# imulki/serenade

Measured on AMD Instinct MI355X. Metric: mel frames/sec converted (UNet ODE + vocoder), 80x1024, higher is better.
Workload: dtype f32

## Files before the change

serenade_amd/csrc/resunit_f32.hip:

```cpp
#include <hip/hip_runtime.h>

#include "common.h"
#include "conv_common.h"
#include "serenade_hip.h"

namespace {

constexpr int HALO_MAX = 50;
constexpr int NTH = 512;

typedef unsigned u32x4r __attribute__((ext_vector_type(4)));

struct FDivR {
  uint32_t mul, shift;
};
__device__ __forceinline__ int fdivr(const int n, const FDivR d) {
  return (int)(((uint64_t)(uint32_t)n * d.mul) >> d.shift);
}

template <int C_>
struct UCfg {
  static constexpr int C = C_, CH = C / 32;
  static constexpr int BMI = C == 32 ? 256 : 128;
  static constexpr int A_ROWS = BMI + HALO_MAX + 2;
  static constexpr int A_PLANE = A_ROWS * 144;
  static constexpr int A_BYTES = CH * A_PLANE;
  static constexpr int UNIT = C * 144;
  static constexpr int G = 9216 / UNIT >= 2 ? 2 : 1;
  static constexpr int STAGE = G * UNIT;
  static constexpr int SMEM = A_BYTES + 2 * STAGE;
  static constexpr int F4R = C / 4, RSTEP = NTH / F4R;
  static constexpr int A_LD = (A_ROWS * F4R + NTH - 1) / NTH;
  static_assert(G * C * 8 == NTH, "one 16-B weight piece per thread per stage");
};

template <class R>
__global__ __launch_bounds__(NTH, 4) void resunit_f32_kernel(const SrnResUnitParams p, const int tiles_per_z,
                                                             const int n_tiles, const FDivR d_tpz) {
  constexpr int C = R::C, CH = R::CH, BMI = R::BMI, G = R::G;
  extern __shared__ __attribute__((aligned(16))) unsigned char smem_u[];
  unsigned char* const sA = smem_u;
  unsigned char* const sW = smem_u + R::A_BYTES;

  const int tid = threadIdx.x;
  const int lane = tid & 63;
  const int wave = __builtin_amdgcn_readfirstlane(tid >> 6);
  const int li = lane & 31;
  const int lh = lane >> 5;
  const int k = p.k, dil = p.dilation, T = p.T;
  const int p2 = (k - 1) / 2, p1 = p2 * dil;
  const int BMo = BMI - (k - 1);
  const int hr = BMI + (k - 1) * dil;
  const int U = k * CH;
  const int S = (U + G - 1) / G;
  const float slope = p.slope;

  const int w_n = (tid % (C * 8)) >> 3;
  const int w_g = tid / (C * 8);
  const int w_voff = w_n * (k * C * 4) + w_g * 128 + (tid & 7) * 16;
  const int w_dst = (w_g * C + w_n) * 144 + (tid & 7) * 16;
  const int w_bytes = C * k * C * 4;
  const __amdgpu_buffer_rsrc_t rs_w1 = __builtin_amdgcn_make_buffer_rsrc(const_cast<float*>(p.w1), 0, w_bytes, 0x00020000);
  const __amdgpu_buffer_rsrc_t rs_w2 = __builtin_amdgcn_make_buffer_rsrc(const_cast<float*>(p.w2), 0, w_bytes, 0x00020000);
  u32x4r wr;
  auto w_load = [&](const int j) {
    if (j >= S) wr = __builtin_amdgcn_raw_buffer_load_b128(rs_w2, w_voff, (j - S) * G * 128, 0);
    else wr = __builtin_amdgcn_raw_buffer_load_b128(rs_w1, w_voff, j * G * 128, 0);
  };
  auto w_store = [&](const int buf) {
    *reinterpret_cast<u32x4r*>(sW + buf * R::STAGE + w_dst) = wr;
  };

  constexpr int A_LD = R::A_LD, F4R = R::F4R, RSTEP = R::RSTEP;
  const int a_f4 = tid % F4R;
  const int a_r0 = tid / F4R;
  const int a_voff = (a_r0 * C + a_f4 * 4) * 4;
  const int a_dst0 = (a_f4 >> 3) * R::A_PLANE + a_r0 * 144 + (a_f4 & 7) * 16;
  u32x4r pa[A_LD];
  auto load_a = [&](const int tile) {
    const int z = fdivr(tile, d_tpz);
    const int t0 = (tile - z * tiles_per_z) * BMo;
    const __amdgpu_buffer_rsrc_t rs_x =
        __builtin_amdgcn_make_buffer_rsrc(const_cast<float*>(p.x + (int64_t)z * p.x_bs), 0, T * C * 4, 0x00020000);
    const int v0 = a_voff + (t0 - p2 - p1) * (C * 4);
#pragma unroll
    for (int j = 0; j < A_LD; ++j) pa[j] = __builtin_amdgcn_raw_buffer_load_b128(rs_x, v0 + j * (RSTEP * C * 4), 0, 0);
  };
  auto stage_a = [&]() {
#pragma unroll
    for (int j = 0; j < A_LD; ++j) {
      if (a_r0 + RSTEP * j < hr) {
        float4 v = __builtin_bit_cast(float4, pa[j]);
        v.x = fmaxf(v.x, v.x * slope);
        v.y = fmaxf(v.y, v.y * slope);
        v.z = fmaxf(v.z, v.z * slope);
        v.w = fmaxf(v.w, v.w * slope);
        *reinterpret_cast<float4*>(sA + a_dst0 + j * RSTEP * 144) = v;
      }
    }
  };

  const int wm0 = (C == 64 ? (wave & 3) : wave) * 32;
  const int ng0 = C == 64 ? (wave >> 2) : 0;
  const int fa_lane = (wm0 + li) * 144 + 16 * lh;
  const int fb_lane = R::A_BYTES + (ng0 * 32 + li) * 144 + 16 * lh;
  f32x16 acc;
  auto zero_acc = [&]() {
#pragma unroll
    for (int r = 0; r < 16; ++r) acc[r] = 0.f;
  };

  auto compute = [&](const int buf, const int u0, const int step) {
#pragma unroll
    for (int g = 0; g < G; ++g) {
      const int u = u0 + g;
      if (u >= U) break;
      const int tap = u / CH;
      const int c = u - tap * CH;
      const float* a = reinterpret_cast<const float*>(smem_u + (fa_lane + (c * R::A_PLANE + tap * step * 144)));
      const float* b = reinterpret_cast<const float*>(smem_u + (fb_lane + (buf * R::STAGE + g * C * 144)));
#pragma unroll
      for (int kk = 0; kk < 4; ++kk) {
        const float4 af = *reinterpret_cast<const float4*>(a + kk * 8);
        const float4 bf = *reinterpret_cast<const float4*>(b + kk * 8);
        acc = __builtin_amdgcn_mfma_f32_32x32x2f32(af.x, bf.x, acc, 0, 0, 0);
        acc = __builtin_amdgcn_mfma_f32_32x32x2f32(af.y, bf.y, acc, 0, 0, 0);
        acc = __builtin_amdgcn_mfma_f32_32x32x2f32(af.z, bf.z, acc, 0, 0, 0);
        acc = __builtin_amdgcn_mfma_f32_32x32x2f32(af.w, bf.w, acc, 0, 0, 0);
      }
    }
  };

  int wj = 0, wbuf = 0;
  auto conv_pass = [&](const int step) {
    for (int s = 0; s < S; ++s) {
      compute(wbuf, s * G, step);
      w_store(wbuf ^ 1);
      int nxt = wj + 2;
      if (nxt >= 2 * S) nxt -= 2 * S;
      w_load(nxt);
      wj = wj + 1 == 2 * S ? 0 : wj + 1;
      wbuf ^= 1;
      __syncthreads();
    }
  };

  int tile = blockIdx.x;
  load_a(tile);
  w_load(0);
  w_store(0);
  w_load(2 * S > 1 ? 1 : 0);

  const float bias1 = p.b1[ng0 * 32 + li];
  const float bias2 = p.b2[ng0 * 32 + li];
  const bool divide = p.post_div != 0.f && p.post_div != 1.f;
  const bool has_q = p.res2 != nullptr;
  const int mid_lane = ng0 * R::A_PLANE + ((wm0 + 4 * lh) * 36 + li) * 4;
  const int io_lane = ((wm0 + 4 * lh) * C + ng0 * 32 + li) * 4;

  for (; tile < n_tiles; tile += gridDim.x) {
    const int z = fdivr(tile, d_tpz);
    const int t0 = (tile - z * tiles_per_z) * BMo;
    stage_a();
    __syncthreads();
    const int next = tile + gridDim.x;
    load_a(next < n_tiles ? next : tile);

    zero_acc();
    conv_pass(dil);
    if (t0 - p2 >= 0 && t0 - p2 + BMI <= T) {
#pragma unroll
      for (int r = 0; r < 16; ++r) {
        const float v = acc[r] + bias1;
        *reinterpret_cast<float*>(sA + mid_lane + ((r & 3) + 8 * (r >> 2)) * 144) = fmaxf(v, v * slope);
      }
    } else {
#pragma unroll
      for (int r = 0; r < 16; ++r) {
        const int dr = (r & 3) + 8 * (r >> 2);
        const int gi = t0 - p2 + wm0 + 4 * lh + dr;
        float v = acc[r] + bias1;
        v = fmaxf(v, v * slope);
        if (gi < 0 || gi >= T) v = 0.f;
        *reinterpret_cast<float*>(sA + mid_lane + dr * 144) = v;
      }
    }
    __syncthreads();

    zero_acc();
    conv_pass(1);

    const int row_end = min(BMo, T - t0);
    const int64_t zoff = (int64_t)t0 * C;
    const int io_bytes = row_end * C * 4;
    const __amdgpu_buffer_rsrc_t rs_xe = __builtin_amdgcn_make_buffer_rsrc(
        const_cast<float*>(p.x + (int64_t)z * p.x_bs + zoff), 0, io_bytes, 0x00020000);
    const __amdgpu_buffer_rsrc_t rs_qe = __builtin_amdgcn_make_buffer_rsrc(
        const_cast<float*>(has_q ? p.res2 + (int64_t)z * p.res2_bs + zoff : p.x), 0, has_q ? io_bytes : 0, 0x00020000);
    const __amdgpu_buffer_rsrc_t rs_oe =
        __builtin_amdgcn_make_buffer_rsrc(p.out + (int64_t)z * p.out_bs + zoff, 0, io_bytes, 0x00020000);
    if (wm0 + 32 <= row_end) {
#pragma unroll
      for (int gq = 0; gq < 4; ++gq) {
        float xv[4], qv[4];
#pragma unroll
        for (int i = 0; i < 4; ++i) {
          xv[i] = __builtin_bit_cast(float, __builtin_amdgcn_raw_buffer_load_b32(rs_xe, io_lane, (8 * gq + i) * C * 4, 0));
          qv[i] = __builtin_bit_cast(float, __builtin_amdgcn_raw_buffer_load_b32(rs_qe, io_lane, (8 * gq + i) * C * 4, 0));
        }
#pragma unroll
        for (int i = 0; i < 4; ++i) {
          float v = acc[4 * gq + i] + bias2 + xv[i];
          if (has_q) v += qv[i];
          if (divide) v = v / p.post_div;
          __builtin_amdgcn_raw_buffer_store_b32(__builtin_bit_cast(unsigned, v), rs_oe, io_lane, (8 * gq + i) * C * 4, 0);
        }
      }
    } else if (wm0 < row_end) {
#pragma unroll
      for (int gq = 0; gq < 4; ++gq) {
        float xv[4], qv[4];
#pragma unroll
        for (int i = 0; i < 4; ++i) {
          xv[i] = __builtin_bit_cast(float, __builtin_amdgcn_raw_buffer_load_b32(rs_xe, io_lane + (8 * gq + i) * C * 4, 0, 0));
          qv[i] = __builtin_bit_cast(float, __builtin_amdgcn_raw_buffer_load_b32(rs_qe, io_lane + (8 * gq + i) * C * 4, 0, 0));
        }
#pragma unroll
        for (int i = 0; i < 4; ++i) {
          float v = acc[4 * gq + i] + bias2 + xv[i];
          if (has_q) v += qv[i];
          if (divide) v = v / p.post_div;
          __builtin_amdgcn_raw_buffer_store_b32(__builtin_bit_cast(unsigned, v), rs_oe, io_lane + (8 * gq + i) * C * 4, 0, 0);
        }
      }
    }
  }
}

FDivR make_fdivr(const uint32_t d) {
  int lg = 0;
  while ((1u << lg) < d) ++lg;
  const int k = 26 + lg;
  return FDivR{(uint32_t)(((1ull << k) + d - 1) / d), (uint32_t)k};
}

template <class R>
int launch_unit(const SrnResUnitParams& p, hipStream_t stream) {
  static SrnSmemAttr smem_attr;
  if (const int e = smem_attr.ensure(reinterpret_cast<const void*>(&resunit_f32_kernel<R>), R::SMEM)) return e;
  const int BMo = R::BMI - (p.k - 1);
  const int tiles_per_z = (p.T + BMo - 1) / BMo;
  const int64_t n_tiles = (int64_t)p.n_batch * tiles_per_z;
  if (n_tiles <= 0 || n_tiles >= (1ll << 26)) return 0;
  const int grid = (int)(n_tiles < 512 ? n_tiles : 512);
  hipLaunchKernelGGL((resunit_f32_kernel<R>), dim3(grid), dim3(NTH), R::SMEM, stream, p, tiles_per_z, (int)n_tiles,
                     make_fdivr((uint32_t)tiles_per_z));
  SRN_CHECK_LAUNCH();
  return 1;
}

}

int srn_resunit_f32_try(const SrnResUnitParams& p, hipStream_t stream) {
  if (!(p.slope >= 0.f && p.slope <= 1.f)) return 0;
  if ((int64_t)p.T * p.C * 4 >= 0x7fffffffll) return 0;
  return p.C == 32 ? launch_unit<UCfg<32>>(p, stream) : launch_unit<UCfg<64>>(p, stream);
}
```

Baseline: 62060.

## Prefetch residual inputs during conv and stage next tile before epilogue stores

The residual and second-residual epilogue loads are now issued before the last two weight stages of the second convolution, so their global-memory latency overlaps with MFMA work. Staging of the next tile's input into shared memory moves ahead of the output stores, and the tile loop is rewritten with an explicit prefetch flag. Splitting out the full and partial-tile epilogues removes a branch, relying on buffer bounds to guard partial rows. The cost is 32 extra live registers across the conv stages, which may reduce occupancy. The loop also now assumes every block starts with a valid tile.

```diff
diff --git a/serenade_amd/csrc/resunit_f32.hip b/serenade_amd/csrc/resunit_f32.hip
--- a/serenade_amd/csrc/resunit_f32.hip
+++ b/serenade_amd/csrc/resunit_f32.hip
@@ -132,17 +132,18 @@
   };
 
   int wj = 0, wbuf = 0;
-  auto conv_pass = [&](const int step) {
-    for (int s = 0; s < S; ++s) {
-      compute(wbuf, s * G, step);
-      w_store(wbuf ^ 1);
-      int nxt = wj + 2;
-      if (nxt >= 2 * S) nxt -= 2 * S;
-      w_load(nxt);
-      wj = wj + 1 == 2 * S ? 0 : wj + 1;
-      wbuf ^= 1;
-      __syncthreads();
-    }
+  auto conv_stage = [&](const int s, const int step) {
+    compute(wbuf, s * G, step);
+    w_store(wbuf ^ 1);
+    int nxt = wj + 2;
+    if (nxt >= 2 * S) nxt -= 2 * S;
+    w_load(nxt);
+    wj = wj + 1 == 2 * S ? 0 : wj + 1;
+    wbuf ^= 1;
+    __syncthreads();
+  };
+  auto conv_pass = [&](const int step, const int s1) {
+    for (int s = 0; s < s1; ++s) conv_stage(s, step);
   };
 
   int tile = blockIdx.x;
@@ -158,16 +159,18 @@
   const int mid_lane = ng0 * R::A_PLANE + ((wm0 + 4 * lh) * 36 + li) * 4;
   const int io_lane = ((wm0 + 4 * lh) * C + ng0 * 32 + li) * 4;
 
-  for (; tile < n_tiles; tile += gridDim.x) {
+  stage_a();
+  __syncthreads();
+
+  for (;;) {
     const int z = fdivr(tile, d_tpz);
     const int t0 = (tile - z * tiles_per_z) * BMo;
-    stage_a();
-    __syncthreads();
     const int next = tile + gridDim.x;
-    load_a(next < n_tiles ? next : tile);
+    const bool more = next < n_tiles;
+    load_a(more ? next : tile);
 
     zero_acc();
-    conv_pass(dil);
+    conv_pass(dil, S);
     if (t0 - p2 >= 0 && t0 - p2 + BMI <= T) {
 #pragma unroll
       for (int r = 0; r < 16; ++r) {
@@ -187,53 +190,46 @@
     }
     __syncthreads();
 
-    zero_acc();
-    conv_pass(1);
-
     const int row_end = min(BMo, T - t0);
     const int64_t zoff = (int64_t)t0 * C;
     const int io_bytes = row_end * C * 4;
-    const __amdgpu_buffer_rsrc_t rs_xe = __builtin_amdgcn_make_buffer_rsrc(
-        const_cast<float*>(p.x + (int64_t)z * p.x_bs + zoff), 0, io_bytes, 0x00020000);
-    const __amdgpu_buffer_rsrc_t rs_qe = __builtin_amdgcn_make_buffer_rsrc(
-        const_cast<float*>(has_q ? p.res2 + (int64_t)z * p.res2_bs + zoff : p.x), 0, has_q ? io_bytes : 0, 0x00020000);
+    float xv[16], qv[16];
+    auto epi_load = [&]() {
+      const __amdgpu_buffer_rsrc_t rs_xe = __builtin_amdgcn_make_buffer_rsrc(
+          const_cast<float*>(p.x + (int64_t)z * p.x_bs + zoff), 0, io_bytes, 0x00020000);
+      const __amdgpu_buffer_rsrc_t rs_qe = __builtin_amdgcn_make_buffer_rsrc(
+          const_cast<float*>(has_q ? p.res2 + (int64_t)z * p.res2_bs + zoff : p.x), 0, has_q ? io_bytes : 0, 0x00020000);
+#pragma unroll
+      for (int r = 0; r < 16; ++r) {
+        const int ro = ((r & 3) + 8 * (r >> 2)) * C * 4;
+        xv[r] = __builtin_bit_cast(float, __builtin_amdgcn_raw_buffer_load_b32(rs_xe, io_lane + ro, 0, 0));
+        qv[r] = __builtin_bit_cast(float, __builtin_amdgcn_raw_buffer_load_b32(rs_qe, io_lane + ro, 0, 0));
+      }
+    };
+
+    zero_acc();
+    conv_pass(1, S - 2);
+    epi_load();
+    if (S >= 2) conv_stage(S - 2, 1);
+    conv_stage(S - 1, 1);
+
+    stage_a();
+#pragma unroll
+    for (int r = 0; r < 16; ++r) {
+      float v = acc[r] + bias2 + xv[r];
+      if (has_q) v += qv[r];
+      if (divide) v = v / p.post_div;
+      xv[r] = v;
+    }
+    __syncthreads();
     const __amdgpu_buffer_rsrc_t rs_oe =
         __builtin_amdgcn_make_buffer_rsrc(p.out + (int64_t)z * p.out_bs + zoff, 0, io_bytes, 0x00020000);
-    if (wm0 + 32 <= row_end) {
-#pragma unroll
-      for (int gq = 0; gq < 4; ++gq) {
-        float xv[4], qv[4];
-#pragma unroll
-        for (int i = 0; i < 4; ++i) {
-          xv[i] = __builtin_bit_cast(float, __builtin_amdgcn_raw_buffer_load_b32(rs_xe, io_lane, (8 * gq + i) * C * 4, 0));
-          qv[i] = __builtin_bit_cast(float, __builtin_amdgcn_raw_buffer_load_b32(rs_qe, io_lane, (8 * gq + i) * C * 4, 0));
-        }
-#pragma unroll
-        for (int i = 0; i < 4; ++i) {
-          float v = acc[4 * gq + i] + bias2 + xv[i];
-          if (has_q) v += qv[i];
-          if (divide) v = v / p.post_div;
-          __builtin_amdgcn_raw_buffer_store_b32(__builtin_bit_cast(unsigned, v), rs_oe, io_lane, (8 * gq + i) * C * 4, 0);
-        }
-      }
-    } else if (wm0 < row_end) {
-#pragma unroll
-      for (int gq = 0; gq < 4; ++gq) {
-        float xv[4], qv[4];
-#pragma unroll
-        for (int i = 0; i < 4; ++i) {
-          xv[i] = __builtin_bit_cast(float, __builtin_amdgcn_raw_buffer_load_b32(rs_xe, io_lane + (8 * gq + i) * C * 4, 0, 0));
-          qv[i] = __builtin_bit_cast(float, __builtin_amdgcn_raw_buffer_load_b32(rs_qe, io_lane + (8 * gq + i) * C * 4, 0, 0));
-        }
-#pragma unroll
-        for (int i = 0; i < 4; ++i) {
-          float v = acc[4 * gq + i] + bias2 + xv[i];
-          if (has_q) v += qv[i];
-          if (divide) v = v / p.post_div;
-          __builtin_amdgcn_raw_buffer_store_b32(__builtin_bit_cast(unsigned, v), rs_oe, io_lane + (8 * gq + i) * C * 4, 0, 0);
-        }
-      }
-    }
+#pragma unroll
+    for (int r = 0; r < 16; ++r)
+      __builtin_amdgcn_raw_buffer_store_b32(__builtin_bit_cast(unsigned, xv[r]), rs_oe,
+                                            io_lane + ((r & 3) + 8 * (r >> 2)) * C * 4, 0, 0);
+    if (!more) break;
+    tile = next;
   }
 }
 
```

Result: no change. 62270, median of 6 (+0.3%).
